# mlysy/rodeo

Measured on AMD Instinct MI355X. Metric: ODE steps/sec x batch (trajectory-steps/s), FitzHugh-Nagumo q=3, 4000 steps, solve_mv, higher is better.
Workload: dtype f64

## Files before the change

rodeo_amd/csrc/solve_tile3.hip:

```cpp
#include <cstdlib>
#include "common.hpp"
#include "kalman_small.hpp"
#include "mfma_tile.hpp"
#include "philox.hpp"
#include "rhs.hpp"
#include "solve_args.hpp"
#include "solve_paths.hpp"
#include "solve_tile3_kernels.hpp"
#include "fenrir_at_args.hpp"

namespace rk {

constexpr int CHUNK = 16;
constexpr int ITEM_BYTES = 3 * 128;
constexpr int BUF_BYTES = CHUNK * 4 * ITEM_BYTES;
constexpr int ZONE_BYTES = 64 * TILE_DOUBLES * 8;

__device__ __forceinline__ int lds_byte(int s, int g, int which, int idx) {
    const int item = s * 4 + g;
    return item * ITEM_BYTES + which * 128 + (tile_slot(s, g, idx) << 3);
}

__device__ __forceinline__ void tile3_gain_producers(const SolveArgs& a, const double* __restrict__ tiles, int D, int tw, int wave,
                                                     int lane, int n_tiles, size_t tstride, int n_chunks, char* lds_raw,
                                                     char* zones) {
    constexpr int P = 3;
    const int p = wave - 1;
    const int s = lane >> 2, g = lane & 3;
    int tau = tw * 4 + g;
    if (tau >= n_tiles) tau = n_tiles - 1;
    const int b = tau / D, blk = tau - b * D;
    double Q[P][P], R[P][P];
    load_block_consts<P>(a, blk, b, Q, R);
    int woff[12];
#pragma unroll
    for (int i = 0; i < 3; ++i)
#pragma unroll
        for (int j = 0; j < 4; ++j) woff[i * 4 + j] = lds_byte(s, g, 0, i * 4 + j);
    char* const zone = zones + p * ZONE_BYTES;
    const unsigned zone_lds = __builtin_amdgcn_readfirstlane(lds_addr(zone));
    int frow[6], fcol[6];
#pragma unroll
    for (int i = 0; i < 6; ++i) { const int j = 64 * i + lane; frow[i] = j / 24; fcol[i] = (j % 24) * 16; }
    const char* const wave_tiles = (const char*)(tiles + (size_t)tw * 4 * TILE_DOUBLES);
    auto fetch = [&](int ch) {
        const int n_hi = a.N - 1 - ch * CHUNK;
#pragma unroll
        for (int i = 0; i < 6; ++i) {
            const int n = n_hi - frow[i];
            lds_dma16(wave_tiles + (size_t)(n < 1 ? 1 : n) * tstride * 8 + fcol[i], zone_lds + 1024 * i);
        }
    };
    lds_dma_wait_all();
    if (p < n_chunks) fetch(p);
    double mf[P], Sf[P][P], mp[P], Sp[P][P], A[P][P], X[P][P], rpiv[P];
    for (int t = -3; t < n_chunks; ++t) {
        const int ch1 = t + 3, ch2 = t + 2, ch3 = t + 1;
        if (ch1 % 3 == p) {
            if (ch1 < n_chunks) {
                lds_dma_wait_all();
                double buf[TILE_DOUBLES];
#pragma unroll
                for (int k = 0; k < 6; ++k) {
                    const double2 v = *(const double2*)(zone + 96 * lane + 16 * k);
                    buf[2 * k] = v.x; buf[2 * k + 1] = v.y;
                }
                lds_reads_done();
                if (ch1 + 3 < n_chunks) fetch(ch1 + 3);
#pragma unroll
                for (int i = 0; i < P; ++i) {
#pragma unroll
                    for (int j = 0; j < P; ++j) Sf[i][j] = buf[i * 4 + j];
                    mf[i] = buf[i * 4 + 3];
                }
                predict_block<P>(Q, R, mf, Sf, mp, Sp);
            }
        } else if (ch2 >= 0 && ch2 % 3 == p) {
            if (ch2 < n_chunks) {
                double T[P][P];
                mm_nt<P, P, P>(Sf, Q, T);
#pragma unroll
                for (int i = 0; i < P; ++i)
#pragma unroll
                    for (int j = 0; j < P; ++j) { A[i][j] = Sp[i][j]; X[i][j] = T[j][i]; }
                lu_factor_fwd<P, P>(A, X, rpiv);
            }
        } else if (ch3 >= 0) {
            if (ch3 < n_chunks) {
                lu_back<P, P>(A, X, rpiv);
                const int n = a.N - 1 - ch3 * CHUNK - s;
                if (n >= 1) {
                    char* o = lds_raw + (ch3 & 1) * BUF_BYTES;
#pragma unroll
                    for (int i = 0; i < P; ++i) {
#pragma unroll
                        for (int j = 0; j < P; ++j) {
                            *(double*)(o + woff[i * 4 + j]) = Sp[i][j];
                            *(double*)(o + woff[i * 4 + j] + 128) = X[i][j];
                            *(double*)(o + woff[i * 4 + j] + 256) = Sf[i][j];
                        }
                        *(double*)(o + woff[i * 4 + 3]) = mp[i];
                        *(double*)(o + woff[i * 4 + 3] + 256) = mf[i];
                    }
                }
            }
        }
        lds_barrier();   
    }
}

__global__ void __launch_bounds__(256) bwd_mv_tile3_kernel(SolveArgs a, double* __restrict__ tiles, int D) {
    __shared__ __attribute__((aligned(16))) char lds_all[2 * BUF_BYTES];
    __shared__ __attribute__((aligned(16))) char zones[3 * ZONE_BYTES];
    const int wave = threadIdx.x >> 6, lane = threadIdx.x & 63;
    const int n_tiles = a.B * D;
    const size_t tstride = (size_t)n_tiles * TILE_DOUBLES;
    const int n_chunks = (a.N - 1 + CHUNK - 1) / CHUNK;

    for (int i = threadIdx.x; i < 2 * 64 * 3 * 16; i += 256) {
        const int idx = i & 15, which = (i >> 4) % 3, item = ((i >> 4) / 3) & 63, buf = i / (64 * 3 * 16);
        const double v = (idx == 15) ? 1.0 : 0.0;
        *(double*)(lds_all + buf * BUF_BYTES + lds_byte(item >> 2, item & 3, which, idx)) = v;
    }
    __syncthreads();

    const int tw = blockIdx.x;
    char* const lds_raw = lds_all;
    double* const dump = tiles + (size_t)(a.N + 1) * tstride + (size_t)tw * 64;
    const int role = wave;

    if (role >= 1) {
        tile3_gain_producers(a, tiles, D, tw, role, lane, n_tiles, tstride, n_chunks, lds_raw, zones);
    } else {
        const TileCoord tc = tile_coord<1>(tw, lane, n_tiles);
        __builtin_amdgcn_s_setprio(3);
        const int r = tc.r, g = tc.g, c = tc.c, idx = r * 4 + c;
        const bool st = tc.valid && r < 3;
        double* base = st ? tiles + (size_t)tc.tau * TILE_DOUBLES + idx : dump + lane;
        const size_t ostride = st ? tstride : 0;
        int roff[4];
#pragma unroll
        for (int k = 0; k < 4; ++k) roff[k] = lds_byte(k, g, 0, idx) - k * 4 * ITEM_BYTES;
        double Ms = st ? base[(size_t)a.N * ostride] : ((r == 3 && c == 3) ? 1.0 : 0.0);
        const char* const wave_rows = (const char*)(tiles + (size_t)tw * 4 * TILE_DOUBLES);
        const size_t row_bytes = tstride * sizeof(double);
        const unsigned bvoff = st ? (unsigned)((g * TILE_DOUBLES + idx) * sizeof(double)) : 0x80000000u;
        const bool buffer_ok = (CHUNK - 1) * row_bytes + 384 < 0x7fffffffull;
        const int chunk_span = (int)((CHUNK - 1) * row_bytes + 384);
        lds_barrier();
        lds_barrier();
        lds_barrier();
        for (int t = 0; t < n_chunks; ++t) {
            const char* in = lds_raw + (t & 1) * BUF_BYTES;
            const int n_hi = a.N - 1 - t * CHUNK;
            const int cnt = __builtin_amdgcn_readfirstlane(n_hi >= CHUNK ? CHUNK : n_hi);
            double* o = base + (size_t)n_hi * ostride;
            {
                if (cnt == CHUNK && buffer_ok) {
                    constexpr int LOOKAHEAD = 4;
                    double Mp[CHUNK], Gt[CHUNK], Mf[CHUNK];
                    auto load = [&](int s) {
                        const char* q = in + roff[s & 3] + s * 4 * ITEM_BYTES;
                        Mp[s] = *(const double*)(q);
                        Gt[s] = *(const double*)(q + 128);
                        Mf[s] = *(const double*)(q + 256);
                    };
#pragma unroll
                    for (int s = 0; s < LOOKAHEAD; ++s) load(s);
                    const __amdgpu_buffer_rsrc_t rsrc = __builtin_amdgcn_make_buffer_rsrc(
                        (void*)(wave_rows + (size_t)(n_hi - (CHUNK - 1)) * row_bytes), 0, chunk_span, 0x00020000);
                    double Dm = Ms - Mp[0];
#pragma unroll
                    for (int s = 0; s < CHUNK; ++s) {
                        if (s + LOOKAHEAD < CHUNK) load(s + LOOKAHEAD);
                        __builtin_amdgcn_sched_barrier(0);
                        const double V1 = MF(Dm, Gt[s], 0.0);
                        Ms = MF(V1, Gt[s], Mf[s]);
                        if (s + 1 < CHUNK) Dm = Ms - Mp[s + 1];
                        u32x2 bits;
                        __builtin_memcpy(&bits, &Ms, 8);
                        __builtin_amdgcn_raw_buffer_store_b64(bits, rsrc, (int)bvoff, (int)((CHUNK - 1 - s) * row_bytes), 0);
                        __builtin_amdgcn_sched_barrier(0);
                    }
                } else {
                    for (int s = 0; s < cnt; ++s) {
                        const char* q = in + lds_byte(s, g, 0, idx);
                        const double Mp = *(const double*)(q), Gt = *(const double*)(q + 128), Mf = *(const double*)(q + 256);
                        const double V1 = MF(Ms - Mp, Gt, 0.0);
                        Ms = MF(V1, Gt, Mf);
                        o[0] = Ms;
                        o -= ostride;
                    }
                }
            }
            lds_barrier();   
        }
    }
}

struct FenrirObs {
    const double *obs, *obs_w, *obs_v;
    const int32_t* obs_ind;
    int n_obs;
    double* logdens;
};

template <bool AT, class OB>
__device__ __forceinline__ void fenrir_tile3_body(const SolveArgs& a, const double* __restrict__ tiles, int D, const OB& ob) {
    __shared__ __attribute__((aligned(16))) char lds_all[2 * BUF_BYTES];
    __shared__ __attribute__((aligned(16))) char zones[3 * ZONE_BYTES];
    const int wave = threadIdx.x >> 6, lane = threadIdx.x & 63;
    const int n_tiles = a.B * D;
    const size_t tstride = (size_t)n_tiles * TILE_DOUBLES;
    const int n_chunks = (a.N - 1 + CHUNK - 1) / CHUNK;

    for (int i = threadIdx.x; i < 2 * 64 * 3 * 16; i += 256) {
        const int idx = i & 15, which = (i >> 4) % 3, item = ((i >> 4) / 3) & 63, buf = i / (64 * 3 * 16);
        const double v = (idx == 15) ? 1.0 : 0.0;
        *(double*)(lds_all + buf * BUF_BYTES + lds_byte(item >> 2, item & 3, which, idx)) = v;
    }
    __syncthreads();

    const int tw = blockIdx.x;
    char* const lds_raw = lds_all;

    if (wave >= 1) {
        tile3_gain_producers(a, tiles, D, tw, wave, lane, n_tiles, tstride, n_chunks, lds_raw, zones);
    } else {
        __builtin_amdgcn_s_setprio(3);
        const int r = lane >> 4, g = (lane >> 2) & 3, c = lane & 3, idx = r * 4 + c;
        const int tau_raw = tw * 4 + g;
        const bool valid = tau_raw < n_tiles;
        const int tau = valid ? tau_raw : n_tiles - 1;
        const int b = tau / D, blk = tau - b * D;
        const bool in_tile = valid && r < 3;
        const double e3 = (r == 3 && c == 3) ? 1.0 : 0.0, I4 = r == c ? 1.0 : 0.0;
        const double* const my = tiles + (size_t)tau * TILE_DOUBLES + idx;
        int roff[4];
#pragma unroll
        for (int k = 0; k < 4; ++k) roff[k] = lds_byte(k, g, 0, idx) - k * 4 * ITEM_BYTES;
        double Ms = in_tile ? my[(size_t)a.N * tstride] : e3;
        double acc = 0.0;
        int i = ob.n_obs - 1;
        int next = -1;
        [[maybe_unused]] int off = 0;
        auto look = [&]() {
            if constexpr (AT) {
                next = i >= 0 ? ob.tab[4 * i] : -1;
                off = i >= 0 ? ob.tab[4 * i + 1] : 0;
            } else {
                next = i >= 0 ? ob.obs_ind[i] : -1;
            }
        };
        look();
        auto observe = [&]() {
            const double xw = valid ? (r < 3 ? ob.obs_w[((size_t)i * D + blk) * 3 + r] : -ob.obs[(size_t)i * D + blk]) : 0.0;
            const double Om = valid ? ob.obs_v[(size_t)i * D + blk] : 1.0;
            double MsT = MF(Ms, I4, 0.0);
            MsT = r == 3 ? 0.0 : MsT;
            const double WS = MF(xw, Ms, 0.0);
            const double Z = MF(MsT, xw, 0.0);
            const double w = MF(Z, xw, 0.0) + Om;
            const double z = -quad_bcast3(WS);
            if (fabs(w) > 1e-8) acc += -0.5 * (z * z / w + log(w)) - 0.5 * 1.83787706640934548356;
            const double K = Z / w;
            Ms = fma(-K, WS, Ms);
            --i;
            look();
        };
        auto step = [&](double Mp, double Gt, double Mf) {
            const double V1 = MF(Ms - Mp, Gt, 0.0);
            Ms = MF(V1, Gt, Mf);
        };
        [[maybe_unused]] auto interval = [&](int n, bool to_node) {
            if constexpr (AT) {
                const double* const my_hops = ob.hops + (size_t)tau * FENRIR_AT_TILE_REC + idx;
                const int n_rec = ob.n_pre + ob.n_post;
                auto hop = [&](int rec) {
                    const double* q = my_hops + (size_t)fenrir_at_clamp(rec, n_rec) * n_tiles * FENRIR_AT_TILE_REC;
                    step(q[0], q[16], q[32]);
                };
                hop(ob.n_pre + fenrir_at_clamp(ob.tab[4 * i + 3], ob.n_post));
                do {
                    const int pre = fenrir_at_clamp(ob.tab[4 * i + 2], ob.n_pre);
                    observe();
                    if (to_node || (off && next == n)) hop(pre);
                } while (off && next == n);
            }
        };
        if (next >= a.N && !off) observe();
        __syncthreads();
        __syncthreads();
        __syncthreads();
        for (int t = 0; t < n_chunks; ++t) {
            const char* in = lds_raw + (t & 1) * BUF_BYTES;
            const int n_hi = a.N - 1 - t * CHUNK;
            const int cnt = __builtin_amdgcn_readfirstlane(n_hi >= CHUNK ? CHUNK : n_hi);
            const bool has_obs = next > n_hi - cnt;
            if (cnt == CHUNK && !has_obs) {
                constexpr int LOOKAHEAD = 4;
                double Mp[CHUNK], Gt[CHUNK], Mf[CHUNK];
                auto load = [&](int s) {
                    const char* q = in + roff[s & 3] + s * 4 * ITEM_BYTES;
                    Mp[s] = *(const double*)(q);
                    Gt[s] = *(const double*)(q + 128);
                    Mf[s] = *(const double*)(q + 256);
                };
#pragma unroll
                for (int s = 0; s < LOOKAHEAD; ++s) load(s);
                double Dm = Ms - Mp[0];
#pragma unroll
                for (int s = 0; s < CHUNK; ++s) {
                    if (s + LOOKAHEAD < CHUNK) load(s + LOOKAHEAD);
                    __builtin_amdgcn_sched_barrier(0);
                    const double V1 = MF(Dm, Gt[s], 0.0);
                    Ms = MF(V1, Gt[s], Mf[s]);
                    if (s + 1 < CHUNK) Dm = Ms - Mp[s + 1];
                    __builtin_amdgcn_sched_barrier(0);
                }
            } else {
                for (int s = 0; s < cnt; ++s) {
                    const int n = n_hi - s;
                    bool hops = false;
                    if constexpr (AT) hops = off && next == n;
                    if (hops) {
                        interval(n, true);
                    } else {
                        const char* q = in + lds_byte(s, g, 0, idx);
                        step(*(const double*)(q), *(const double*)(q + 128), *(const double*)(q + 256));
                    }
                    if (!off && next == n) observe();
                }
            }
            __syncthreads();
        }
        if constexpr (AT)
            if (off && next == 0) interval(0, false);
        if (!off && next == 0) {
            Ms = in_tile ? my[0] : e3;
            observe();
        }
        if (valid && r == 0 && c == 0) atomicAdd(&ob.logdens[b], acc);
    }
}

__global__ void __launch_bounds__(256) fenrir_bwd_tile3_kernel(SolveArgs a, const double* __restrict__ tiles, int D, FenrirObs ob) {
    fenrir_tile3_body<false>(a, tiles, D, ob);
}

__global__ void __launch_bounds__(256) fenrir_bwd_at_tile3_kernel(SolveArgs a, const double* __restrict__ tiles, int D, FenrirAt ob) {
    fenrir_tile3_body<true>(a, tiles, D, ob);
}

constexpr int SIM_ITEM = 256;
constexpr int SIM_BUF = CHUNK * 4 * SIM_ITEM;

__device__ __forceinline__ int sim_tile_byte(int s, int g, int idx) {
    const int item = s * 4 + g;
    return item * SIM_ITEM + (tile_slot(s, g, idx) << 3);
}
__device__ __forceinline__ int sim_vec_byte(int s, int g, int which, int rr) {
    const int item = s * 4 + g;
    return item * SIM_ITEM + 128 + (vec_slot(s, g, which, rr) << 3);
}

struct SimLogpost {
    const double* obs;
    const int32_t* obs_ind;
    int n_obs;
    double noise_sd;
    const double* upars;
    int n_prior;
    double prior_sd;
    double* logpost;
};
constexpr int LP_MAX_OBS = 512, LP_MAX_VALS = 1024;

template <bool LP>
__global__ void __launch_bounds__(256, 2) bwd_sim_tile3_kernel(SolveArgs a, double* __restrict__ tiles, int D, SimLogpost lp) {
    constexpr int P = 3;
    __shared__ double lp_obs[LP ? LP_MAX_VALS : 1];
    __shared__ int lp_ind[LP ? LP_MAX_OBS : 1];
    if constexpr (LP) {
        for (int i = threadIdx.x; i < lp.n_obs * D; i += 256) lp_obs[i] = lp.obs[i];
        for (int i = threadIdx.x; i < lp.n_obs; i += 256) { const int ni = lp.obs_ind[i]; lp_ind[i] = ni < 0 ? 0 : (ni > a.N ? a.N : ni); }
    }
    __shared__ __attribute__((aligned(16))) char lds_all[2 * SIM_BUF];
    __shared__ __attribute__((aligned(16))) char zones[3 * ZONE_BYTES];
    constexpr int QR_STRIDE = 2 * 9 + 2;
    __shared__ __attribute__((aligned(16))) double qr[4 * QR_STRIDE];
    const int wave = threadIdx.x >> 6, lane = threadIdx.x & 63;
    const int n_tiles = a.B * D;
    const size_t tstride = (size_t)n_tiles * TILE_DOUBLES;
    const int n_chunks = (a.N + CHUNK - 1) / CHUNK;
    for (int i = threadIdx.x; i < 2 * SIM_BUF / 8; i += 256) ((double*)lds_all)[i] = 0.0;
    __syncthreads();
    const int tw = blockIdx.x;
    char* const lds_raw = lds_all;
    double* const dump = tiles + (size_t)(a.N + 1) * tstride + (size_t)tw * 64;

    if (wave >= 1) {
        const int p = wave - 1;
        const int s = lane >> 2, g = lane & 3;
        int tau = tw * 4 + g;
        if (tau >= n_tiles) tau = n_tiles - 1;
        const int b = tau / D, blk = tau - b * D;
        const uint32_t traj = (uint32_t)(a.traj_offset + (uint64_t)b);
        if (p == 0 && s == 0) {
            double Q0[P][P], R0[P][P];
            load_block_consts<P>(a, blk, b, Q0, R0);
#pragma unroll
            for (int i = 0; i < P; ++i)
#pragma unroll
                for (int j = 0; j < P; ++j) { qr[g * QR_STRIDE + i * P + j] = Q0[i][j]; qr[g * QR_STRIDE + 9 + i * P + j] = R0[i][j]; }
        }
        lds_barrier();
        const double* const my_qr = qr + g * QR_STRIDE;
        auto load_q = [&](double (&Qv)[P][P]) {
#pragma unroll
            for (int i = 0; i < P; ++i)
#pragma unroll
                for (int j = 0; j < P; ++j) Qv[i][j] = my_qr[i * P + j];
        };
        int woff[9], voff[3], voff1[3];
#pragma unroll
        for (int i = 0; i < 3; ++i) {
#pragma unroll
            for (int j = 0; j < 3; ++j) woff[i * 3 + j] = sim_tile_byte(s, g, i * 4 + j);
            voff[i] = sim_vec_byte(s, g, 0, i);
            voff1[i] = sim_vec_byte(s, g, 1, i);
        }
        char* const zone = zones + p * ZONE_BYTES;
        const unsigned zone_lds = __builtin_amdgcn_readfirstlane(lds_addr(zone));
        int frow[6], fcol[6];
#pragma unroll
        for (int i = 0; i < 6; ++i) { const int j = 64 * i + lane; frow[i] = j / 24; fcol[i] = (j % 24) * 16; }
        const char* const wave_tiles = (const char*)(tiles + (size_t)tw * 4 * TILE_DOUBLES);
        auto fetch = [&](int ch) {
            const int n_hi = a.N - ch * CHUNK;
#pragma unroll
            for (int i = 0; i < 6; ++i) {
                const int n = n_hi - frow[i];
                lds_dma16(wave_tiles + (size_t)(n < 1 ? 1 : n) * tstride * 8 + fcol[i], zone_lds + 1024 * i);
            }
        };
        lds_dma_wait_all();
        if (p < n_chunks) fetch(p);
        double mf[P], Sf[P][P], mp[P], Sp[P][P], T[P][P], A[P][P], X[P][P], rpiv[P], z[P];
        for (int t = -3; t < n_chunks; ++t) {
            const int ch1 = t + 3, ch2 = t + 2, ch3 = t + 1;
            if (ch1 % 3 == p) {
                if (ch1 < n_chunks) {
                    lds_dma_wait_all();
                    double buf[TILE_DOUBLES];
#pragma unroll
                    for (int k = 0; k < 6; ++k) {
                        const double2 v = *(const double2*)(zone + 96 * lane + 16 * k);
                        buf[2 * k] = v.x; buf[2 * k + 1] = v.y;
                    }
                    lds_reads_done();
                    if (ch1 + 3 < n_chunks) fetch(ch1 + 3);
#pragma unroll
                    for (int i = 0; i < P; ++i) {
#pragma unroll
                        for (int j = 0; j < P; ++j) Sf[i][j] = buf[i * 4 + j];
                        mf[i] = buf[i * 4 + 3];
                    }
                    {
                        double Q[P][P], R[P][P];
                        load_q(Q);
#pragma unroll
                        for (int i = 0; i < P; ++i)
#pragma unroll
                            for (int j = 0; j < P; ++j) R[i][j] = my_qr[9 + i * P + j];
                        predict_block<P>(Q, R, mf, Sf, mp, Sp);
                    }
                    const int n = a.N - ch1 * CHUNK - s;
#ifdef RK_T3_ABLATE_SIMZ
                    z[0] = 0.25 + 1e-3 * n; z[1] = -0.5;
#else
                    normal_pair(a.seed, traj, (uint32_t)(n < 1 ? 1 : n), (uint32_t)blk, PURPOSE_SMOOTH, 0u, z[0], z[1]);
#endif
                }
            } else if (ch2 >= 0 && ch2 % 3 == p) {
                if (ch2 < n_chunks) {
                    {
                        double Q[P][P];
                        load_q(Q);
                        mm_nt<P, P, P>(Sf, Q, T);
                    }
#pragma unroll
                    for (int i = 0; i < P; ++i)
#pragma unroll
                        for (int j = 0; j < P; ++j) { A[i][j] = Sp[i][j]; X[i][j] = T[j][i]; }
                    lu_factor_fwd<P, P>(A, X, rpiv);
                    const int n = a.N - ch2 * CHUNK - s;
                    double z3;
#ifdef RK_T3_ABLATE_SIMZ
                    z[2] = 0.125 + 1e-3 * n; z3 = 0.0;
#else
                    normal_pair(a.seed, traj, (uint32_t)(n < 1 ? 1 : n), (uint32_t)blk, PURPOSE_SMOOTH, 1u, z[2], z3);
#endif
                }
            } else if (ch3 >= 0) {
                if (ch3 < n_chunks) {
                    const int n = a.N - ch3 * CHUNK - s;
                    double GT[P][P], Ssim[P][P], L[P][P], G[P][P];
                    lu_back<P, P>(A, X, rpiv);
                    const bool term = n == a.N;
#pragma unroll
                    for (int i = 0; i < P; ++i)
#pragma unroll
                        for (int j = 0; j < P; ++j) G[i][j] = term ? 0.0 : X[j][i];
                    mm_nt<P, P, P>(G, T, GT);
#pragma unroll
                    for (int i = 0; i < P; ++i)
#pragma unroll
                        for (int j = 0; j < P; ++j) Ssim[i][j] = Sf[i][j] - GT[i][j];
#ifdef RK_T3_ABLATE_SIMPSD
#pragma unroll
                    for (int i = 0; i < P; ++i)
#pragma unroll
                        for (int j = 0; j < P; ++j) L[i][j] = Ssim[i][j];
#else
                    psd_factor<P>(Ssim, L);
#endif
                    if (n >= 1) {
                        char* o = lds_raw + (ch3 & 1) * SIM_BUF;
#pragma unroll
                        for (int i = 0; i < P; ++i) {
                            double w = mf[i];
#pragma unroll
                            for (int k = 0; k <= i; ++k) w = fma(L[i][k], z[k], w);
#pragma unroll
                            for (int j = 0; j < P; ++j) *(double*)(o + woff[i * 3 + j]) = G[j][i];
                            *(double*)(o + voff[i]) = term ? 0.0 : mp[i];
                            *(double*)(o + voff1[i]) = w;
                        }
                    }
                }
            }
            lds_barrier();
        }
    } else {
        const TileCoord tc = tile_coord<1>(tw, lane, n_tiles);
        const int r = tc.r, g = tc.g, c = tc.c, idx = r * 4 + c;
        const int b = tc.tau / D, blk = tc.tau - b * D;
        const bool st = tc.valid && r < 3 && c == 0 && a.x != nullptr;
        const size_t xstride = (size_t)D * P * a.B;
        double* bx = st ? a.x + ((size_t)blk * P + r) * a.B + b : dump + lane;
        const double LOG_SQRT_2PI = 0.91893853320467274178;
        const double lsd = LP ? log(lp.noise_sd) : 0.0;
        int io = LP ? lp.n_obs - 1 : -1;
        double acc = 0.0;
        auto next_index = [&]() { return io >= 0 ? __builtin_amdgcn_readfirstlane(lp_ind[io]) : -1; };
        auto observe = [&](double xv) {
            const double zz = (lp_obs[io * D + blk] - xv) / lp.noise_sd;
            acc += -0.5 * zz * zz - lsd - LOG_SQRT_2PI;
            --io;
        };
        const size_t sx = st ? xstride : 0;
        const bool xbuf_ok = (size_t)CHUNK * xstride * sizeof(double) < 0x7fffffffull;
        const int xvo = st && xbuf_ok ? (int)((((size_t)blk * P + r) * a.B + b) * sizeof(double)) : (int)0x80000000;
        int roff[4], rvec[4], rvec1[4];
#pragma unroll
        for (int k = 0; k < 4; ++k) {
            roff[k] = sim_tile_byte(k, g, idx) - k * 4 * SIM_ITEM;
            rvec[k] = sim_vec_byte(k, g, 0, r) - k * 4 * SIM_ITEM;
            rvec1[k] = sim_vec_byte(k, g, 1, r) - k * 4 * SIM_ITEM;
        }
        double x = 0.0;
        lds_barrier();
        int next_n = LP ? next_index() : -1;
        lds_barrier();
        lds_barrier();
        lds_barrier();
        for (int t = 0; t < n_chunks; ++t) {
            const char* in = lds_raw + (t & 1) * SIM_BUF;
            const int n_hi = a.N - t * CHUNK;
            const int cnt = __builtin_amdgcn_readfirstlane(n_hi >= CHUNK ? CHUNK : n_hi);
            double* o = bx + (size_t)n_hi * sx;
            auto step = [&](const char* q, const char* qv, const char* qw) {
                const double Gt = *(const double*)(q), mp = *(const double*)(qv), mfw = *(const double*)(qw);
                x = MF(Gt, x - mp, mfw);
                o[0] = x;
                o -= sx;
            };
            int n_cur = n_hi;
            if (cnt == CHUNK && xbuf_ok) {
                const __amdgpu_buffer_rsrc_t rsrc = __builtin_amdgcn_make_buffer_rsrc(
                    (void*)(a.x + (size_t)(n_hi - (CHUNK - 1)) * xstride), 0, (int)(CHUNK * xstride * sizeof(double)), 0x00020000);
                double xs[LP ? CHUNK : 1];
#pragma unroll
                for (int s = 0; s < CHUNK; ++s) {
                    const double Gt = *(const double*)(in + roff[s & 3] + s * 4 * SIM_ITEM);
                    const double mp = *(const double*)(in + rvec[s & 3] + s * 4 * SIM_ITEM);
                    const double mfw = *(const double*)(in + rvec1[s & 3] + s * 4 * SIM_ITEM);
                    x = MF(Gt, x - mp, mfw);
                    u32x2 bits;
                    __builtin_memcpy(&bits, &x, 8);
                    __builtin_amdgcn_raw_buffer_store_b64(bits, rsrc, xvo, (int)((CHUNK - 1 - s) * xstride * sizeof(double)), 0);
                    if constexpr (LP) xs[s] = x;
                }
                if constexpr (LP) {
                    if (next_n > n_hi - CHUNK) {
#pragma unroll
                        for (int s = 0; s < CHUNK; ++s)
                            while (n_hi - s == next_n) { observe(xs[s]); next_n = next_index(); }
                    }
                }
            } else if (cnt == CHUNK) {
#pragma unroll
                for (int s = 0; s < CHUNK; ++s) {
                    step(in + roff[s & 3] + s * 4 * SIM_ITEM, in + rvec[s & 3] + s * 4 * SIM_ITEM, in + rvec1[s & 3] + s * 4 * SIM_ITEM);
                    if constexpr (LP) {
                        while (n_cur == next_n) { observe(x); next_n = next_index(); }
                    }
                    --n_cur;
                }
            } else {
                for (int s = 0; s < cnt; ++s) {
                    step(in + sim_tile_byte(s, g, idx), in + sim_vec_byte(s, g, 0, r), in + sim_vec_byte(s, g, 1, r));
                    if constexpr (LP) {
                        while (n_cur == next_n) { observe(x); next_n = next_index(); }
                    }
                    --n_cur;
                }
            }
            lds_barrier();
        }
        const double x_init = tiles[(size_t)tc.tau * TILE_DOUBLES + r * 4 + 3];
        if (st) bx[0] = x_init;
        if constexpr (LP) {
            while (next_n == 0) { observe(x_init); next_n = next_index(); }
            if (D >= 2) acc += __shfl_xor(acc, 4, 64);
            if (D >= 4) acc += __shfl_xor(acc, 8, 64);
            if (tc.valid && r == 0 && c == 0 && blk == 0) {
                if (lp.upars) {
                    const double lps = log(lp.prior_sd);
                    for (int k = 0; k < lp.n_prior; ++k) {
                        const double zz = lp.upars[(size_t)k * a.B + b] / lp.prior_sd;
                        acc += -0.5 * zz * zz - lps - LOG_SQRT_2PI;
                    }
                }
                lp.logpost[b] = acc;
            }
        }
    }
}

template <class RHS>
static int launch_fwd_tile(rk_handle h, const rk_solve_cfg* c, const SolveArgs& a, double* tiles) {
    const LaunchGeom g = fwd_tile_geom(a.B, RHS::D);
    launch_placement_primer(h, g.grid, g.block);
    LaunchTimer t(h, "fwd_tile3_kernel");
    const bool ok = dispatch_int<RK_INTERROGATE_RODEO, RK_INTERROGATE_CHKREBTII>(c->interrogate, [&](auto I) {
        hipLaunchKernelGGL((fwd_tile3_kernel<RHS, I>), g.grid, g.block, 0, h->stream, a, tiles);
    });
    RK_REQUIRE(ok, RK_ERR_UNSUPPORTED, "tile path: interrogate id %d not supported", c->interrogate);
    t.stop();
    RK_HIP(hipGetLastError());
    return RK_OK;
}

template <int D>
constexpr bool tile_geom_matches() {
    if constexpr (D == 0) return true;
    else return tiles_per_wave(D) == Tpw<D>::value && tile_waves(D) == TileWaves<D>::value && tile_geom_matches<D - 1>();
}
static_assert(tile_geom_matches<TILE_MAX_BLOCKS>(), "tiles_per_wave / tile_waves differ from Tpw<D> / TileWaves<D>");

bool tile3_supported(const rk_solve_cfg* c, int mode) {
    if (c->flags & (RK_FLAG_STORE_PRED | RK_FLAG_BATCH_MINOR)) return false;
    if (c->kalman_type != RK_KALMAN_STANDARD || c->n_bstate != 3 || c->n_bmeas != 1) return false;
    if (c->interrogate < RK_INTERROGATE_RODEO || c->interrogate > RK_INTERROGATE_CHKREBTII) return false;
    if (is_user_rhs(c->rhs_id)) return user_tile_available(c, JIT_TILE3);
    return builtin_has_n_block(c->rhs_id, c->n_block);
}

bool tile3_sim_logpost_supported(const rk_solve_cfg* c, int n_obs) {
    return tile3_supported(c, RK_MODE_SIM) && (c->n_block == 1 || c->n_block == 2 || c->n_block == 4) && n_obs <= LP_MAX_OBS &&
           n_obs * c->n_block <= LP_MAX_VALS;
}

int tile3_solve_sim_logpost(rk_handle h, const rk_solve_cfg* c, const SolveArgs& a, double* tiles, const double* obs,
                            const int32_t* obs_ind, int n_obs, double noise_sd, const double* upars, int n_prior, double prior_sd,
                            double* logpost) {
    SimLogpost lp;
    lp.obs = obs; lp.obs_ind = obs_ind; lp.n_obs = n_obs; lp.noise_sd = noise_sd; lp.upars = upars; lp.n_prior = n_prior;
    lp.prior_sd = prior_sd; lp.logpost = logpost;
    return tile3_solve(h, c, a, tiles, RK_MODE_SIM, &lp);
}

int tile3_solve(rk_handle h, const rk_solve_cfg* c, const SolveArgs& a, double* tiles, int mode, const SimLogpost* lp) {
    int rc = RK_ERR_UNSUPPORTED;
    if (is_user_rhs(c->rhs_id)) rc = user_forward_tile(h, c, a, tiles, JIT_TILE3);
    else with_builtin_rhs(c->rhs_id, [&](auto rhs) { rc = launch_fwd_tile<decltype(rhs)>(h, c, a, tiles); });
    if (rc || mode == RK_MODE_FILTER) return rc;
    return tile3_backward(h, a, tiles, mode, lp);
}

int tile3_backward(rk_handle h, const SolveArgs& a, double* tiles, int mode, const SimLogpost* lp) {
    if (mode == RK_MODE_SIM) {
        LaunchTimer t(h, "bwd_sim_tile3_kernel");
        if (lp) hipLaunchKernelGGL(bwd_sim_tile3_kernel<true>, dim3(div_up(a.B * a.D, 4)), dim3(256), 0, h->stream, a, tiles, a.D, *lp);
        else hipLaunchKernelGGL(bwd_sim_tile3_kernel<false>, dim3(div_up(a.B * a.D, 4)), dim3(256), 0, h->stream, a, tiles, a.D, SimLogpost{});
        t.stop();
        RK_HIP(hipGetLastError());
        return RK_OK;
    }
    if (a.N < 2) return RK_OK;
    LaunchTimer t(h, "bwd_mv_tile3_kernel");
    hipLaunchKernelGGL(bwd_mv_tile3_kernel, dim3(div_up(a.B * a.D, 4)), dim3(256), 0, h->stream, a, tiles, a.D);
    t.stop();
    RK_HIP(hipGetLastError());
    return RK_OK;
}

int tile3_fenrir_backward(rk_handle h, const SolveArgs& a, const double* tiles, const double* obs, const double* obs_w,
                          const double* obs_v, const int32_t* obs_ind, int n_obs, double* logdens) {
    FenrirObs ob;
    ob.obs = obs; ob.obs_w = obs_w; ob.obs_v = obs_v; ob.obs_ind = obs_ind; ob.n_obs = n_obs; ob.logdens = logdens;
    LaunchTimer t(h, "fenrir_bwd_tile3_kernel");
    hipLaunchKernelGGL(fenrir_bwd_tile3_kernel, dim3(div_up(a.B * a.D, 4)), dim3(256), 0, h->stream, a, tiles, a.D, ob);
    t.stop();
    RK_HIP(hipGetLastError());
    return RK_OK;
}

int tile3_fenrir_backward_at(rk_handle h, const SolveArgs& a, const double* tiles, const FenrirAt& ob) {
    LaunchTimer t(h, "fenrir_bwd_at_tile3_kernel");
    hipLaunchKernelGGL(fenrir_bwd_at_tile3_kernel, dim3(div_up(a.B * a.D, 4)), dim3(256), 0, h->stream, a, tiles, a.D, ob);
    t.stop();
    RK_HIP(hipGetLastError());
    return RK_OK;
}

}
```

Baseline: 5.957 billion.

## Split LDS staging into planes, compile-time buffer offsets, windowed buffer-store descriptors

```diff
diff --git a/rodeo_amd/csrc/solve_tile3.hip b/rodeo_amd/csrc/solve_tile3.hip
--- a/rodeo_amd/csrc/solve_tile3.hip
+++ b/rodeo_amd/csrc/solve_tile3.hip
@@ -1,4 +1,5 @@
 #include <cstdlib>
+#include <type_traits>
 #include "common.hpp"
 #include "kalman_small.hpp"
 #include "mfma_tile.hpp"
@@ -11,14 +12,36 @@
 
 namespace rk {
 
+#ifdef RK_T3_STAMPS
+#define T3_STAMPS_BEGIN() long long st_acc_[3] = {0, 0, 0}, st_t_ = __builtin_amdgcn_s_memtime()
+#define T3_STAMP(k) do { const long long now_ = __builtin_amdgcn_s_memtime(); st_acc_[k] += now_ - st_t_; st_t_ = now_; } while (0)
+#define T3_STAMPS_END(tail, wave, lane) do { if ((lane) == 0) for (int k_ = 0; k_ < 3; ++k_) (tail)[4 * (wave) + k_] = (double)st_acc_[k_]; } while (0)
+#else
+#define T3_STAMPS_BEGIN() do {} while (0)
+#define T3_STAMP(k) do {} while (0)
+#define T3_STAMPS_END(tail, wave, lane) do {} while (0)
+#endif
+
 constexpr int CHUNK = 16;
-constexpr int ITEM_BYTES = 3 * 128;
-constexpr int BUF_BYTES = CHUNK * 4 * ITEM_BYTES;
+constexpr int STEP_BYTES = 4 * 128;
+constexpr int PLANE_BYTES = CHUNK * STEP_BYTES;
+constexpr int BUF_BYTES = 3 * PLANE_BYTES;
 constexpr int ZONE_BYTES = 64 * TILE_DOUBLES * 8;
 
 __device__ __forceinline__ int lds_byte(int s, int g, int which, int idx) {
-    const int item = s * 4 + g;
-    return item * ITEM_BYTES + which * 128 + (tile_slot(s, g, idx) << 3);
+    return which * PLANE_BYTES + (s * 4 + g) * 128 + (tile_slot(s, g, idx) << 3);
+}
+
+__device__ __forceinline__ void chain_bases(int g, int idx, int (&roff)[4]) {
+#pragma unroll
+    for (int k = 0; k < 4; ++k) roff[k] = lds_byte(k, g, 0, idx) - k * STEP_BYTES;
+}
+template <int BUF>
+__device__ __forceinline__ void load_item(const char* lds_raw, const int (&roff)[4], int s, double& Mp, double& Gt, double& Mf) {
+    const char* q = lds_raw + roff[s & 3] + (BUF * BUF_BYTES + s * STEP_BYTES);
+    Mp = *(const double*)(q);
+    Gt = *(const double*)(q + PLANE_BYTES);
+    Mf = *(const double*)(q + 2 * PLANE_BYTES);
 }
 
 __device__ __forceinline__ void tile3_gain_producers(const SolveArgs& a, const double* __restrict__ tiles, int D, int tw, int wave,
@@ -54,11 +77,14 @@
     lds_dma_wait_all();
     if (p < n_chunks) fetch(p);
     double mf[P], Sf[P][P], mp[P], Sp[P][P], A[P][P], X[P][P], rpiv[P];
+    T3_STAMPS_BEGIN();
     for (int t = -3; t < n_chunks; ++t) {
         const int ch1 = t + 3, ch2 = t + 2, ch3 = t + 1;
         if (ch1 % 3 == p) {
             if (ch1 < n_chunks) {
+                T3_STAMP(0);
                 lds_dma_wait_all();
+                T3_STAMP(2);
                 double buf[TILE_DOUBLES];
 #pragma unroll
                 for (int k = 0; k < 6; ++k) {
@@ -96,17 +122,20 @@
 #pragma unroll
                         for (int j = 0; j < P; ++j) {
                             *(double*)(o + woff[i * 4 + j]) = Sp[i][j];
-                            *(double*)(o + woff[i * 4 + j] + 128) = X[i][j];
-                            *(double*)(o + woff[i * 4 + j] + 256) = Sf[i][j];
+                            *(double*)(o + woff[i * 4 + j] + PLANE_BYTES) = X[i][j];
+                            *(double*)(o + woff[i * 4 + j] + 2 * PLANE_BYTES) = Sf[i][j];
                         }
                         *(double*)(o + woff[i * 4 + 3]) = mp[i];
-                        *(double*)(o + woff[i * 4 + 3] + 256) = mf[i];
-                    }
-                }
-            }
-        }
-        lds_barrier();   
+                        *(double*)(o + woff[i * 4 + 3] + 2 * PLANE_BYTES) = mf[i];
+                    }
+                }
+            }
+        }
+        T3_STAMP(0);
+        lds_barrier();
+        T3_STAMP(1);
     }
+    T3_STAMPS_END(const_cast<double*>(tiles) + (size_t)(a.N + 1) * tstride + (size_t)tw * 64, wave, lane);
 }
 
 __global__ void __launch_bounds__(256) bwd_mv_tile3_kernel(SolveArgs a, double* __restrict__ tiles, int D) {
@@ -139,62 +168,72 @@
         double* base = st ? tiles + (size_t)tc.tau * TILE_DOUBLES + idx : dump + lane;
         const size_t ostride = st ? tstride : 0;
         int roff[4];
-#pragma unroll
-        for (int k = 0; k < 4; ++k) roff[k] = lds_byte(k, g, 0, idx) - k * 4 * ITEM_BYTES;
+        chain_bases(g, idx, roff);
         double Ms = st ? base[(size_t)a.N * ostride] : ((r == 3 && c == 3) ? 1.0 : 0.0);
         const char* const wave_rows = (const char*)(tiles + (size_t)tw * 4 * TILE_DOUBLES);
         const size_t row_bytes = tstride * sizeof(double);
-        const unsigned bvoff = st ? (unsigned)((g * TILE_DOUBLES + idx) * sizeof(double)) : 0x80000000u;
-        const bool buffer_ok = (CHUNK - 1) * row_bytes + 384 < 0x7fffffffull;
-        const int chunk_span = (int)((CHUNK - 1) * row_bytes + 384);
-        lds_barrier();
-        lds_barrier();
-        lds_barrier();
-        for (int t = 0; t < n_chunks; ++t) {
-            const char* in = lds_raw + (t & 1) * BUF_BYTES;
-            const int n_hi = a.N - 1 - t * CHUNK;
-            const int cnt = __builtin_amdgcn_readfirstlane(n_hi >= CHUNK ? CHUNK : n_hi);
-            double* o = base + (size_t)n_hi * ostride;
-            {
-                if (cnt == CHUNK && buffer_ok) {
-                    constexpr int LOOKAHEAD = 4;
-                    double Mp[CHUNK], Gt[CHUNK], Mf[CHUNK];
-                    auto load = [&](int s) {
-                        const char* q = in + roff[s & 3] + s * 4 * ITEM_BYTES;
-                        Mp[s] = *(const double*)(q);
-                        Gt[s] = *(const double*)(q + 128);
-                        Mf[s] = *(const double*)(q + 256);
-                    };
-#pragma unroll
-                    for (int s = 0; s < LOOKAHEAD; ++s) load(s);
-                    const __amdgpu_buffer_rsrc_t rsrc = __builtin_amdgcn_make_buffer_rsrc(
-                        (void*)(wave_rows + (size_t)(n_hi - (CHUNK - 1)) * row_bytes), 0, chunk_span, 0x00020000);
-                    double Dm = Ms - Mp[0];
-#pragma unroll
-                    for (int s = 0; s < CHUNK; ++s) {
-                        if (s + LOOKAHEAD < CHUNK) load(s + LOOKAHEAD);
-                        __builtin_amdgcn_sched_barrier(0);
-                        const double V1 = MF(Dm, Gt[s], 0.0);
-                        Ms = MF(V1, Gt[s], Mf[s]);
-                        if (s + 1 < CHUNK) Dm = Ms - Mp[s + 1];
-                        u32x2 bits;
-                        __builtin_memcpy(&bits, &Ms, 8);
-                        __builtin_amdgcn_raw_buffer_store_b64(bits, rsrc, (int)bvoff, (int)((CHUNK - 1 - s) * row_bytes), 0);
-                        __builtin_amdgcn_sched_barrier(0);
-                    }
-                } else {
-                    for (int s = 0; s < cnt; ++s) {
-                        const char* q = in + lds_byte(s, g, 0, idx);
-                        const double Mp = *(const double*)(q), Gt = *(const double*)(q + 128), Mf = *(const double*)(q + 256);
-                        const double V1 = MF(Ms - Mp, Gt, 0.0);
-                        Ms = MF(V1, Gt, Mf);
-                        o[0] = Ms;
-                        o -= ostride;
-                    }
-                }
-            }
-            lds_barrier();   
-        }
+        const int bvoff = st ? (int)((g * TILE_DOUBLES + idx) * sizeof(double)) : (int)0x80000000;
+        constexpr uint32_t SLICE = 4 * TILE_DOUBLES * sizeof(double), WIN_MAX = 0x7fffffffu - SLICE;
+        const int win_chunks = row_bytes <= WIN_MAX ? (int)(WIN_MAX / (uint32_t)row_bytes) / CHUNK : 0;
+        const int n_full = win_chunks ? (a.N - 1) / CHUNK : 0;
+        const uint32_t row32 = (uint32_t)row_bytes;
+        __amdgpu_buffer_rsrc_t rsrc = __builtin_amdgcn_make_buffer_rsrc((void*)wave_rows, 0, 0, 0x00020000);
+        uint32_t soff = 0;
+        auto open_window = [&](int t) {
+            const int t1 = n_full - t < win_chunks ? n_full : t + win_chunks;
+            soff = (uint32_t)((t1 - t) * CHUNK - 1) * row32;
+            rsrc = __builtin_amdgcn_make_buffer_rsrc((void*)(wave_rows + (size_t)(a.N - t1 * CHUNK) * row_bytes), 0,
+                                                     (int)(soff + SLICE), 0x00020000);
+            return t1;
+        };
+        auto full_chunk = [&](auto buf) __attribute__((always_inline)) {
+            constexpr int BUF = decltype(buf)::value, LOOKAHEAD = 4;
+            double Mp[CHUNK], Gt[CHUNK], Mf[CHUNK];
+#pragma unroll
+            for (int s = 0; s < LOOKAHEAD; ++s) load_item<BUF>(lds_raw, roff, s, Mp[s], Gt[s], Mf[s]);
+            double Dm = Ms - Mp[0];
+#pragma unroll
+            for (int s = 0; s < CHUNK; ++s) {
+                if (s + LOOKAHEAD < CHUNK) load_item<BUF>(lds_raw, roff, s + LOOKAHEAD, Mp[s + LOOKAHEAD], Gt[s + LOOKAHEAD], Mf[s + LOOKAHEAD]);
+                __builtin_amdgcn_sched_barrier(0);
+                const double V1 = MF(Dm, Gt[s], 0.0);
+                Ms = MF(V1, Gt[s], Mf[s]);
+                if (s + 1 < CHUNK) Dm = Ms - Mp[s + 1];
+                u32x2 bits;
+                __builtin_memcpy(&bits, &Ms, 8);
+                __builtin_amdgcn_raw_buffer_store_b64(bits, rsrc, bvoff, (int)soff, 0);
+                soff -= row32;
+                __builtin_amdgcn_sched_barrier(0);
+            }
+        };
+        lds_barrier();
+        lds_barrier();
+        lds_barrier();
+        T3_STAMPS_BEGIN();
+        for (int t = 0, t_win = 0; t < n_chunks; ++t) {
+            if (t < n_full) {
+                if (t == t_win) t_win = open_window(t);
+                if (t & 1) full_chunk(std::integral_constant<int, 1>{});
+                else full_chunk(std::integral_constant<int, 0>{});
+            } else {
+                const char* in = lds_raw + (t & 1) * BUF_BYTES;
+                const int n_hi = a.N - 1 - t * CHUNK;
+                const int cnt = __builtin_amdgcn_readfirstlane(n_hi >= CHUNK ? CHUNK : n_hi);
+                double* o = base + (size_t)n_hi * ostride;
+                for (int s = 0; s < cnt; ++s) {
+                    const char* q = in + lds_byte(s, g, 0, idx);
+                    const double Mp = *(const double*)(q), Gt = *(const double*)(q + PLANE_BYTES), Mf = *(const double*)(q + 2 * PLANE_BYTES);
+                    const double V1 = MF(Ms - Mp, Gt, 0.0);
+                    Ms = MF(V1, Gt, Mf);
+                    o[0] = Ms;
+                    o -= ostride;
+                }
+            }
+            T3_STAMP(0);
+            lds_barrier();
+            T3_STAMP(1);
+        }
+        T3_STAMPS_END(dump, 0, lane);
     }
 }
 
@@ -237,8 +276,7 @@
         const double e3 = (r == 3 && c == 3) ? 1.0 : 0.0, I4 = r == c ? 1.0 : 0.0;
         const double* const my = tiles + (size_t)tau * TILE_DOUBLES + idx;
         int roff[4];
-#pragma unroll
-        for (int k = 0; k < 4; ++k) roff[k] = lds_byte(k, g, 0, idx) - k * 4 * ITEM_BYTES;
+        chain_bases(g, idx, roff);
         double Ms = in_tile ? my[(size_t)a.N * tstride] : e3;
         double acc = 0.0;
         int i = ob.n_obs - 1;
@@ -288,6 +326,22 @@
                 } while (off && next == n);
             }
         };
+        auto full_chunk = [&](auto buf) __attribute__((always_inline)) {
+            constexpr int BUF = decltype(buf)::value, LOOKAHEAD = 4;
+            double Mp[CHUNK], Gt[CHUNK], Mf[CHUNK];
+#pragma unroll
+            for (int s = 0; s < LOOKAHEAD; ++s) load_item<BUF>(lds_raw, roff, s, Mp[s], Gt[s], Mf[s]);
+            double Dm = Ms - Mp[0];
+#pragma unroll
+            for (int s = 0; s < CHUNK; ++s) {
+                if (s + LOOKAHEAD < CHUNK) load_item<BUF>(lds_raw, roff, s + LOOKAHEAD, Mp[s + LOOKAHEAD], Gt[s + LOOKAHEAD], Mf[s + LOOKAHEAD]);
+                __builtin_amdgcn_sched_barrier(0);
+                const double V1 = MF(Dm, Gt[s], 0.0);
+                Ms = MF(V1, Gt[s], Mf[s]);
+                if (s + 1 < CHUNK) Dm = Ms - Mp[s + 1];
+                __builtin_amdgcn_sched_barrier(0);
+            }
+        };
         if (next >= a.N && !off) observe();
         __syncthreads();
         __syncthreads();
@@ -298,26 +352,8 @@
             const int cnt = __builtin_amdgcn_readfirstlane(n_hi >= CHUNK ? CHUNK : n_hi);
             const bool has_obs = next > n_hi - cnt;
             if (cnt == CHUNK && !has_obs) {
-                constexpr int LOOKAHEAD = 4;
-                double Mp[CHUNK], Gt[CHUNK], Mf[CHUNK];
-                auto load = [&](int s) {
-                    const char* q = in + roff[s & 3] + s * 4 * ITEM_BYTES;
-                    Mp[s] = *(const double*)(q);
-                    Gt[s] = *(const double*)(q + 128);
-                    Mf[s] = *(const double*)(q + 256);
-                };
-#pragma unroll
-                for (int s = 0; s < LOOKAHEAD; ++s) load(s);
-                double Dm = Ms - Mp[0];
-#pragma unroll
-                for (int s = 0; s < CHUNK; ++s) {
-                    if (s + LOOKAHEAD < CHUNK) load(s + LOOKAHEAD);
-                    __builtin_amdgcn_sched_barrier(0);
-                    const double V1 = MF(Dm, Gt[s], 0.0);
-                    Ms = MF(V1, Gt[s], Mf[s]);
-                    if (s + 1 < CHUNK) Dm = Ms - Mp[s + 1];
-                    __builtin_amdgcn_sched_barrier(0);
-                }
+                if (t & 1) full_chunk(std::integral_constant<int, 1>{});
+                else full_chunk(std::integral_constant<int, 0>{});
             } else {
                 for (int s = 0; s < cnt; ++s) {
                     const int n = n_hi - s;
@@ -327,7 +363,7 @@
                         interval(n, true);
                     } else {
                         const char* q = in + lds_byte(s, g, 0, idx);
-                        step(*(const double*)(q), *(const double*)(q + 128), *(const double*)(q + 256));
+                        step(*(const double*)(q), *(const double*)(q + PLANE_BYTES), *(const double*)(q + 2 * PLANE_BYTES));
                     }
                     if (!off && next == n) observe();
                 }
```

After: 5.967 billion, median of 2. No clear change (+0.2%).
